# pennucci/PulsePortraiture

Measured on AMD Instinct MI355X. Metric: subint_fits_per_sec, higher is better.
Workload: dtype f64

## Files before the change

### pulseportraiture_amd/csrc/pp_fftq.h

```cpp
#pragma once
#include "pp_fft.h"

namespace pp {

__device__ __forceinline__ void lane_swap32(double& a, double& b) {
    unsigned alo = (unsigned)__double2loint(a), ahi = (unsigned)__double2hiint(a);
    unsigned blo = (unsigned)__double2loint(b), bhi = (unsigned)__double2hiint(b);
    auto r0 = __builtin_amdgcn_permlane32_swap(alo, blo, false, false);
    auto r1 = __builtin_amdgcn_permlane32_swap(ahi, bhi, false, false);
    a = __hiloint2double((int)r1[0], (int)r0[0]);
    b = __hiloint2double((int)r1[1], (int)r0[1]);
}
__device__ __forceinline__ void lane_swap16(double& a, double& b) {
    unsigned alo = (unsigned)__double2loint(a), ahi = (unsigned)__double2hiint(a);
    unsigned blo = (unsigned)__double2loint(b), bhi = (unsigned)__double2hiint(b);
    auto r0 = __builtin_amdgcn_permlane16_swap(alo, blo, false, false);
    auto r1 = __builtin_amdgcn_permlane16_swap(ahi, bhi, false, false);
    a = __hiloint2double((int)r1[0], (int)r0[0]);
    b = __hiloint2double((int)r1[1], (int)r0[1]);
}

__device__ __forceinline__ int fftq_lambda(int t) { return 4 * (t >> 4) + (t & 3) + 16 * ((t >> 2) & 3); }
__device__ __forceinline__ int fftq_lane_of(int lam) { return 16 * ((lam >> 2) & 3) + (lam & 3) + 4 * ((lam >> 4) & 3); }

constexpr int FFTQ_LDS_ELEMS = 4 * 272;

template <int WHEN = 0, typename Mid>
__device__ __forceinline__ void fftq1024(cplx (&v)[16], cplx* lds, const cplx t1, const cplx t2, int tid,
                                         double* power, Mid mid) {
    dft16_first(v);
    if (WHEN == 0) mid();
    dft16_second(v);
    {
        cplx wq[16];
        wq[1] = t1;
#pragma unroll
        for (int j = 2; j < 16; ++j) {
            if (j % 2 == 0) {
                const cplx h = wq[j / 2];
                wq[j] = make_double2(fma(h.x, h.x, -h.y * h.y), 2.0 * h.x * h.y);
            } else wq[j] = cmul(wq[j - 1], wq[1]);
        }
#pragma unroll
        for (int j = 1; j < 16; ++j) v[j] = cmul(v[j], wq[j]);
    }
    if (WHEN == 1) mid();
#pragma unroll
    for (int j = 0; j < 8; ++j) {
        lane_swap32(v[j].x, v[j + 8].x);
        lane_swap32(v[j].y, v[j + 8].y);
    }
#pragma unroll
    for (int j = 0; j < 16; ++j) {
        if (j & 4) continue;
        lane_swap16(v[j].x, v[j + 4].x);
        lane_swap16(v[j].y, v[j + 4].y);
    }
    if (WHEN == 2) mid();
    dft16_first(v);
    {
        const cplx w2 = make_double2(fma(t2.x, t2.x, -t2.y * t2.y), 2.0 * t2.x * t2.y);
        const cplx w3 = cmul(w2, t2);
#pragma unroll
        for (int c = 0; c < 4; ++c) {
            v[4 + c] = cmul(v[4 + c], t2);
            v[8 + c] = cmul(v[8 + c], w2);
            v[12 + c] = cmul(v[12 + c], w3);
        }
    }
    {
        cplx* wbase = lds + (tid >> 4) * 272 + 17 * (tid & 15);
#pragma unroll
        for (int j = 0; j < 16; ++j) wbase[j] = v[j];
        lds_sync<64>();
        const cplx* rbase = lds + (tid >> 4) * 272 + (tid & 15);
#pragma unroll
        for (int j = 0; j < 16; ++j) v[j] = rbase[17 * j];
        lds_sync<64>();
    }
    if (WHEN == 3) mid();
    dft_reg<16>(v);
    if (power) {
        double acc = 0.0;
#pragma unroll
        for (int j = 0; j < 16; ++j) {
            if (j == 0 && tid == 0) { const double dM = v[0].x - v[0].y; acc += dM * dM; }
            else acc += cnorm(v[j]);
        }
        *power += acc;
    }
}

__device__ __forceinline__ int fftq512_lambda(int t) {
    return 4 * ((t >> 5) & 1) + 2 * ((t >> 4) & 1) + 32 * ((t >> 3) & 1) + 16 * ((t >> 2) & 1) + 8 * ((t >> 1) & 1) + (t & 1);
}
__device__ __forceinline__ int fftq512_lane_of(int lam) {
    return 32 * ((lam >> 2) & 1) + 16 * ((lam >> 1) & 1) + 8 * ((lam >> 5) & 1) + 4 * ((lam >> 4) & 1) + 2 * ((lam >> 3) & 1) + (lam & 1);
}
constexpr int FFTQ512_LDS_ELEMS = 8 * 72;

__device__ __forceinline__ double lane_xor8(double v) {
    int lo = __double2loint(v), hi = __double2hiint(v);
    lo = __builtin_amdgcn_update_dpp(lo, lo, 0x128, 0xF, 0xF, false);
    hi = __builtin_amdgcn_update_dpp(hi, hi, 0x128, 0xF, 0xF, false);
    return __hiloint2double(hi, lo);
}

template <int WHEN = 0, typename Mid>
__device__ __forceinline__ void fftq512(cplx (&v)[8], cplx* lds, const cplx t1, const cplx t2, const cplx t3, int tid,
                                        double* power, Mid mid) {
    dft_reg<8>(v);
    if (WHEN == 0) mid();
    {
        cplx wq[8];
        wq[1] = t1;
#pragma unroll
        for (int j = 2; j < 8; ++j) {
            if (j % 2 == 0) {
                const cplx h = wq[j / 2];
                wq[j] = make_double2(fma(h.x, h.x, -h.y * h.y), 2.0 * h.x * h.y);
            } else wq[j] = cmul(wq[j - 1], wq[1]);
        }
#pragma unroll
        for (int j = 1; j < 8; ++j) v[j] = cmul(v[j], wq[j]);
    }
#pragma unroll
    for (int j = 0; j < 4; ++j) {
        lane_swap32(v[j].x, v[j + 4].x);
        lane_swap32(v[j].y, v[j + 4].y);
    }
#pragma unroll
    for (int j = 0; j < 8; ++j) {
        if (j & 2) continue;
        lane_swap16(v[j].x, v[j + 2].x);
        lane_swap16(v[j].y, v[j + 2].y);
    }
    dft4(v[0], v[2], v[4], v[6]);
    dft4(v[1], v[3], v[5], v[7]);
    {
        const cplx w2 = make_double2(fma(t2.x, t2.x, -t2.y * t2.y), 2.0 * t2.x * t2.y);
        const cplx w3 = cmul(w2, t2);
#pragma unroll
        for (int c = 0; c < 2; ++c) {
            v[2 + c] = cmul(v[2 + c], t2);
            v[4 + c] = cmul(v[4 + c], w2);
            v[6 + c] = cmul(v[6 + c], w3);
        }
    }
    {
        const bool up = (tid & 8) != 0;
        const double sg = up ? -1.0 : 1.0;
        const cplx w = up ? t3 : make_double2(1.0, 0.0);
#pragma unroll
        for (int j = 0; j < 8; ++j) {
            const cplx p = make_double2(lane_xor8(v[j].x), lane_xor8(v[j].y));
            const cplx d = make_double2(fma(sg, v[j].x, p.x), fma(sg, v[j].y, p.y));
            v[j] = cmul(d, w);
        }
    }
    {
        cplx* wbase = lds + (tid >> 3) * 72 + 9 * (tid & 7);
#pragma unroll
        for (int j = 0; j < 8; ++j) wbase[j] = v[j];
        lds_sync<64>();
        const cplx* rbase = lds + (tid >> 3) * 72 + (tid & 7);
#pragma unroll
        for (int j = 0; j < 8; ++j) v[j] = rbase[9 * j];
        lds_sync<64>();
    }
    if (WHEN == 3) mid();
    dft_reg<8>(v);
    if (power) {
        double acc = 0.0;
#pragma unroll
        for (int j = 0; j < 8; ++j) {
            if (j == 0 && tid == 0) { const double dM = v[0].x - v[0].y; acc += dM * dM; }
            else acc += cnorm(v[j]);
        }
        *power += acc;
    }
}

template <int M> struct FftQ;
template <> struct FftQ<1024> {
    static constexpr int R = 16, LDS_ELEMS = FFTQ_LDS_ELEMS;
    static __device__ __forceinline__ int lambda(int t) { return fftq_lambda(t); }
    static __device__ __forceinline__ int lane_of(int lam) { return fftq_lane_of(lam); }
    template <int WHEN, typename Mid>
    static __device__ __forceinline__ void run(cplx (&v)[16], cplx* lds, const cplx* twB, int tid, double* power, Mid mid) {
        const cplx t1 = twB[2 * tid], t2 = twB[32 * (tid & 15)];
        fftq1024<WHEN>(v, lds, t1, t2, tid, power, mid);
    }
};
template <> struct FftQ<512> {
    static constexpr int R = 8, LDS_ELEMS = FFTQ512_LDS_ELEMS;
    static __device__ __forceinline__ int lambda(int t) { return fftq512_lambda(t); }
    static __device__ __forceinline__ int lane_of(int lam) { return fftq512_lane_of(lam); }
    template <int WHEN, typename Mid>
    static __device__ __forceinline__ void run(cplx (&v)[8], cplx* lds, const cplx* twB, int tid, double* power, Mid mid) {
        const cplx t1 = twB[2 * tid], t2 = twB[16 * (tid & 15)], t3 = twB[64 * (tid & 7)];
        fftq512<WHEN>(v, lds, t1, t2, t3, tid, power, mid);
    }
};

}
```

### pulseportraiture_amd/csrc/pp_xspec1024q.h

```cpp
#pragma once
#ifndef PP_TAIL_M_LDS
#define PP_TAIL_M_LDS 1
#endif
#ifndef PP_MAIN_M_LDS
#define PP_MAIN_M_LDS 0
#endif
#include "pp_fftq.h"

#ifndef PP_SLOT_EARLY_EXIT
#define PP_SLOT_EARLY_EXIT 1
#endif
#ifndef PP_TICKET_SPREAD
#define PP_TICKET_SPREAD 0
#endif
#ifndef PP_TICKET_WINDOW_NUM
#define PP_TICKET_WINDOW_NUM 3u
#define PP_TICKET_WINDOW_DEN 4u
#endif
#ifndef PP_TAIL_HOOKS
#define PP_TAIL_HOOKS 1
#endif
#ifndef PP_SLOT_PUBLISH_KEPT
#define PP_SLOT_PUBLISH_KEPT 0
#endif

namespace pp {

constexpr bool Q_SPLIT_PREFETCH = true, Q_TW_RELOAD = true;
constexpr int Q_PREFETCH_F64 = 1, Q_PREFETCH_F32 = 0;
template <typename Tin, bool TAIL>
__global__ __launch_bounds__(64, 2) void k_xspec_q1024(XspecArgs a) {
    constexpr int M = 1024, T = 64, R1 = 16, PER1 = 1;
    constexpr int NSL = 7;
    typedef typename RawOf<Tin>::type Raw;
    constexpr int NRED = PP_TSTRIDE + (TAIL ? 2 : 1);
    static_assert(NRED <= 16, "wave_reduce_lds takes 16 values");
    static_assert(PP_TJ == 10, "power ladder written for order 10");
    constexpr int WRED = PP_WRED_DOUBLES(NRED) / 2;
    constexpr int LDSN = WRED > FFTQ_LDS_ELEMS ? WRED : FFTQ_LDS_ELEMS;
    static_assert(2 * LDSN >= PP_TAIL_LDS_DOUBLES, "tail_work's layout of this kernel's LDS");
    constexpr int NML = ((PP_TAIL_M_LDS && TAIL) || (PP_MAIN_M_LDS && !TAIL)) && sizeof(Tin) == 8 ? 2 : 0;
    __shared__ cplx lds[LDSN + 64 * NML];
    cplx* const ldsm = lds + LDSN + threadIdx.x;
    int tid = threadIdx.x;
    const long long nrows = (long long)a.nsub * a.nchan;
    Raw cur[PER1][R1];
    constexpr bool TWR = Q_TW_RELOAD && sizeof(Tin) == 8;
    cplx t1 = a.twB[2 * tid], t2 = a.twB[32 * (tid & 15)];
    const int lam0 = fftq_lambda(tid);
    cplx wb0 = a.twB[lam0 ? lam0 : 64];
    const cplx wbT = a.twB[64];
    int tail_after = 0x7fffffff;
    if (PP_TAIL_HOOKS && a.tail) {
        const unsigned share = (unsigned)(nrows / (long long)gridDim.x) + 1u;
        tail_after = 1 + (int)(((blockIdx.x * 2654435761u) >> 8) % (share * PP_TICKET_WINDOW_NUM / PP_TICKET_WINDOW_DEN + 1u));
#if PP_TICKET_SPREAD
        {
            const unsigned nt = (unsigned)a.tail_nsub;
            const unsigned div = nt ? gridDim.x / nt : 1u;
            if (div > 1u && (((blockIdx.x * 2246822519u) >> 11) % div) != 0u) tail_after = 0x7fffffff;
        }
#endif
    }
    RowWalk<true> rw;
    rw.start(nrows, a.mwords, a.ticket, a.ticket_base);
    long long row = rw.row;
    int n = 0, i = 0;
    if (rw.more) {
        n = __builtin_amdgcn_readfirstlane((int)(row / a.nsub));
        i = __builtin_amdgcn_readfirstlane((int)(row % a.nsub));
        const size_t rc = (size_t)sub_of(a.act, i) * a.nchan_full + (a.coff + n * a.cstep);
        stage_load_global<M, T, R1>(cur, reinterpret_cast<const Tin*>(a.data) + rc * (2 * M), tid);
    }
    cplx mv2[NSL];
    const cplx* mheld = nullptr;
    const cplx* mrow = nullptr;
    int n_held = -1, ktn = 0;
    int i_nx = i, n_nx = n;
#pragma unroll 1
    for (int phase = 0; phase < 2; ++phase) {
    if (phase == 1) {
        if (!(PP_TAIL_HOOKS && a.tail)) break;
        tail_work(a.tail, reinterpret_cast<double*>(lds), 2 * (LDSN + 64 * NML), tid, 1);
        tail_after = 0x7fffffff;
    }
    for (; rw.more && tail_after != 0; rw.advance(), row = rw.row, i = i_nx, n = n_nx, --tail_after) {
        rw.draw(a.ticket);
        rw.peek(nrows, a.ticket_base, a.mwords);
        asm volatile("" : "+v"(tid));
        const int lam = fftq_lambda(tid);
        const bool l0 = (lam == 0);
        const int kb = l0 ? 64 : lam;
        if (TWR) {
            t1 = as_global(a.twB)[2 * tid];
            t2 = as_global(a.twB)[32 * (tid & 15)];
            wb0 = as_global(a.twB)[kb];
        } else {
            asm volatile("" : "+v"(t1.x), "+v"(t1.y), "+v"(t2.x), "+v"(t2.y), "+v"(wb0.x), "+v"(wb0.y));
        }
        const int ia = sub_of(a.act, i), ne = a.coff + n * a.cstep;
        const size_t rc = (size_t)ia * a.nchan_full + ne;
        if (channel_lookup(a, ia, n, ne, M, n_held, mrow, ktn) && mrow != mheld) {
#pragma unroll
            for (int j = 0; j < NSL; ++j) {
                const cplx mval = mrow[kb + 64 * j - 1];
                if (j < NSL - NML) mv2[j] = mval; else ldsm[64 * (j - (NSL - NML))] = mval;
            }
            mheld = mrow;
        }
        const double phin = a.ph0[rc];
        double sd = 0.0;
        cplx v[R1];
#pragma unroll
        for (int k = 0; k < R1; ++k) v[k] = to_cplx(cur[0][k]);
        constexpr bool HALVES = Q_SPLIT_PREFETCH && sizeof(Tin) == 8;
        const Tin* nxrow = nullptr;
        auto load_some = [&](int k0, int k1) {
            const char* gb = reinterpret_cast<const char*>(nxrow);
            const unsigned boff = (unsigned)tid * (unsigned)sizeof(Raw);
#pragma unroll
            for (int k = 0; k < R1; ++k)
                if (k >= k0 && k < k1)
                    cur[0][k] = load_row_once<Raw>(gb + (size_t)(k * 64) * sizeof(Raw) + boff);
        };
#ifndef PP_NEXT_IN_LAMBDA
        rw.next(i, n, i_nx, n_nx, nrows, a.nsub, a.ticket_base, a.ticket, a.mwords);
        {
            const size_t rn = rw.more_nx
                ? (size_t)sub_of(a.act, i_nx) * a.nchan_full + (a.coff + n_nx * a.cstep) : rc;
            nxrow = reinterpret_cast<const Tin*>(a.data) + rn * (2 * M);
        }
#endif
        auto prefetch = [&]() {
            __builtin_amdgcn_sched_barrier(0);
#ifdef PP_NEXT_IN_LAMBDA
            rw.next(i, n, i_nx, n_nx, nrows, a.nsub, a.ticket_base, a.ticket, a.mwords);
            const size_t rn = rw.more_nx
                ? (size_t)sub_of(a.act, i_nx) * a.nchan_full + (a.coff + n_nx * a.cstep) : rc;
            nxrow = reinterpret_cast<const Tin*>(a.data) + rn * (2 * M);
#endif
            load_some(0, HALVES ? R1 / 2 : R1);
            __builtin_amdgcn_sched_barrier(0);
        };
        fftq1024<(sizeof(Tin) == 8 ? Q_PREFETCH_F64 : Q_PREFETCH_F32)>(v, lds, t1, t2, tid, &sd, prefetch);
        __builtin_amdgcn_sched_barrier(0);
        {
            cplx* pub = lds + tid;
            const int nk = PP_SLOT_PUBLISH_KEPT ? max(1, min(NSL, __builtin_amdgcn_readfirstlane(ktn) >> 6)) : NSL;
            switch (NSL - nk) {
                case 0: pub[64 * 0] = v[9];  [[fallthrough]];
                case 1: pub[64 * 1] = v[10]; [[fallthrough]];
                case 2: pub[64 * 2] = v[11]; [[fallthrough]];
                case 3: pub[64 * 3] = v[12]; [[fallthrough]];
                case 4: pub[64 * 4] = v[13]; [[fallthrough]];
                case 5: pub[64 * 5] = v[14]; [[fallthrough]];
                default: pub[64 * 6] = v[15];
            }
            static_assert(NSL == 7, "the run of stores above is written for seven slots");
            if (TAIL) {
#pragma unroll
                for (int r = 0; r < 5; ++r) pub[64 * (NSL + r)] = v[r];
            }
            lds_sync<T>();
        }
        double tail = 0.0;
        if (TAIL) {
            const double h = 0.70710678118654752440;
            const cplx* pt = lds + fftq_lane_of((64 - lam) & 63) + (l0 ? 64 : 0);
            cplx wt = l0 ? make_double2(-h, -h) : cmul(wb0, make_double2(-h, -h));
#pragma unroll
            for (int kd = 12; kd < 16; ++kd) {
                const cplx zk = v[kd];
                cplx zc = pt[64 * (NSL + 15 - kd)];
                zc.y = -zc.y;
                const cplx E = make_double2(zk.x + zc.x, zk.y + zc.y);
                const cplx O = make_double2(zk.x - zc.x, zk.y - zc.y);
                const cplx wo = cmul(wt, O);
                tail += cnorm(make_double2(E.x + wo.y, E.y - wo.x));
                wt = cmul(wt, wbT);
            }
            tail *= 0.25;
            if (tid == 0) { const double dM = v[0].x - v[0].y; tail += dM * dM; }
        }
        if (HALVES) {
            __builtin_amdgcn_sched_barrier(0);
            load_some(R1 / 2, R1);
            __builtin_amdgcn_sched_barrier(0);
        }
        const cplx* pc = lds + fftq_lane_of((64 - lam) & 63);
        const cplx el = unit_phasor<true>((double)kb, phin);
        const cplx wst = make_double2(bcast_lane0(el.x), bcast_lane0(el.y));
        cplx e = el, wb = wb0;
        const int ktu = __builtin_amdgcn_readfirstlane(ktn);
        const double kap0 = PP_TWO_PI * (double)kb;
        double tm[PP_TSTRIDE];
        cplx zc_nx = pc[64 * 6];
#pragma unroll
        for (int j = 0; j < NSL; ++j) {
            if (PP_SLOT_EARLY_EXIT && j > 0 && !(64 * j < ktu)) break;
            cplx zc = zc_nx;
            if (j + 1 < NSL && (!PP_SLOT_EARLY_EXIT || 64 * (j + 1) < ktu)) zc_nx = pc[64 * (5 - j)];
            if (j == 0 || 64 * j < ktu) {
                const cplx zk = csel(l0, v[j + 1], v[j]);
                zc.y = -zc.y;
                const cplx E = make_double2(zk.x + zc.x, zk.y + zc.y);
                const cplx O = make_double2(zk.x - zc.x, zk.y - zc.y);
                const cplx wo = cmul(wb, O);
                const cplx mj = (j < NSL - NML) ? mv2[j < NSL - NML ? j : 0] : ldsm[64 * (j - (NSL - NML))];
                const cplx x = cmulc(make_double2(E.x + wo.y, E.y - wo.x), mj);
                const cplx z = cmul(x, e);
                const double kap = j == 0 ? kap0 : kap0 + kconst<true>(PP_TWO_PI * (double)(64 * j));
                const double p2 = kap * kap, p4 = p2 * p2, p6 = p4 * p2, p8 = p4 * p4, p10 = p8 * p2;
                const double ui = z.y * kap;
                const double ax = fabs(x.x) + fabs(x.y);
                if (j == 0) {
                    tm[0] = z.x;
                    tm[1] = ui;
                    tm[2] = p2 * z.x;
                    tm[3] = p2 * ui;
                    tm[4] = p4 * z.x;
                    tm[5] = p4 * ui;
                    tm[6] = p6 * z.x;
                    tm[7] = p6 * ui;
                    tm[8] = p8 * z.x;
                    tm[9] = p8 * ui;
                    tm[10] = p10 * z.x;
                    tm[11] = (p10 * kap) * ax;
                } else {
                    tm[0] += z.x;
                    tm[1] += ui;
                    tm[2] = fma(p2, z.x, tm[2]);
                    tm[3] = fma(p2, ui, tm[3]);
                    tm[4] = fma(p4, z.x, tm[4]);
                    tm[5] = fma(p4, ui, tm[5]);
                    tm[6] = fma(p6, z.x, tm[6]);
                    tm[7] = fma(p6, ui, tm[7]);
                    tm[8] = fma(p8, z.x, tm[8]);
                    tm[9] = fma(p8, ui, tm[9]);
                    tm[10] = fma(p10, z.x, tm[10]);
                    tm[11] = fma(p10 * kap, ax, tm[11]);
                }
            }
            if (!PP_SLOT_EARLY_EXIT || (j + 1 < NSL && 64 * (j + 1) < ktu)) {
                wb = cmul(wb, wbT);
                e = cmul(e, wst);
            }
        }
        double tr[NRED];
#pragma unroll
        for (int j = 0; j < PP_TSTRIDE; ++j) tr[j] = tm[j];
        tr[PP_TSTRIDE] = sd;
        if (TAIL) tr[NRED - 1] = tail;
        lds_sync<T>();
        double tv = wave_reduce_lds(tr, tid, reinterpret_cast<double*>(lds));
        if ((tid & 3) == 0) {
            const int q = wave_reduce16_index(tid);
            if (q < PP_TSTRIDE) {
                tv *= 0.5;
                a.tay[tay_idx(rc, q)] = (q <= PP_TJ && ((q & 3) == 1 || (q & 3) == 2)) ? -tv : tv;
            }
        }
        if (tid == 4 * PP_TSTRIDE) a.sdraw[rc] = tv;
        if (TAIL && tid == 4 * (PP_TSTRIDE + 1)) {
            constexpr int H = M + 1, kc = (int)(0.75 * H);
            a.noise[rc] = sqrt(tv / (2.0 * M) / (double)(H - kc));
        }
        lds_sync<T>();
    }
    }
    if (PP_TAIL_HOOKS && a.tail) tail_work(a.tail, reinterpret_cast<double*>(lds), 2 * (LDSN + 64 * NML), tid, 1 << 30);
}


#ifndef PP_QF512_HOLD_TEMPLATE
#define PP_QF512_HOLD_TEMPLATE 1
#endif
#ifndef PP_QF512_WPS
#define PP_QF512_WPS 3
#endif
template <int M, typename Tin, bool TAIL>
__global__ __launch_bounds__(64, (M == 1024 ? 2 : PP_QF512_WPS)) void k_xspec_qf(XspecArgs a) {
    typedef FftQ<M> Q;
    constexpr int T = 64, R1 = Q::R, PER1 = 1;
    constexpr int NSL = R1;
    constexpr int JT = (3 * NSL) / 4;
    static_assert((int)(0.75 * (M + 1)) == 64 * JT, "the noise tail starts on a slot boundary");
    typedef typename RawOf<Tin>::type Raw;
    constexpr int NRED = PP_TSTRIDE + (TAIL ? 2 : 1);
    constexpr int WRED = PP_WRED_DOUBLES(NRED) / 2;
    constexpr int LDSN0 = Q::LDS_ELEMS > 64 * NSL ? Q::LDS_ELEMS : 64 * NSL;
    constexpr int LDSN = WRED > LDSN0 ? WRED : LDSN0;
    static_assert(M != 1024 || 2 * LDSN >= PP_TAIL_LDS_DOUBLES, "tail_work's layout of this kernel's LDS");
    __shared__ cplx lds[LDSN];
    int tid = threadIdx.x;
    const long long nrows = (long long)a.nsub * a.nchan;
    Raw cur[PER1][R1];
    const cplx wbT = a.twB[64];
    int tail_after = 0x7fffffff;
    if (PP_TAIL_HOOKS && M == 1024 && a.tail) {
        const unsigned share = (unsigned)(nrows / (long long)gridDim.x) + 1u;
        tail_after = 1 + (int)(((blockIdx.x * 2654435761u) >> 8) % (share * PP_TICKET_WINDOW_NUM / PP_TICKET_WINDOW_DEN + 1u));
    }
    RowWalk<true> rw;
    rw.start(nrows, a.mwords, a.ticket, a.ticket_base);
    long long row = rw.row;
    int n = 0, i = 0;
    if (rw.more) {
        n = __builtin_amdgcn_readfirstlane((int)(row / a.nsub));
        i = __builtin_amdgcn_readfirstlane((int)(row % a.nsub));
        const size_t rc = (size_t)sub_of(a.act, i) * a.nchan_full + (a.coff + n * a.cstep);
        stage_load_global<M, T, R1>(cur, reinterpret_cast<const Tin*>(a.data) + rc * (2 * M), tid);
    }
    int i_nx = i, n_nx = n;
    const cplx* mrow = nullptr;
    int n_held = -1, ktn = 0;
    constexpr bool MHOLD = PP_QF512_HOLD_TEMPLATE && M == 512;
    cplx mv[NSL];
    const cplx* mheld = nullptr;
#pragma unroll 1
    for (int phase = 0; phase < 2; ++phase) {
    if (phase == 1) {
        if (!(PP_TAIL_HOOKS && M == 1024 && a.tail)) break;
        tail_work(a.tail, reinterpret_cast<double*>(lds), 2 * LDSN, tid, 1);
        tail_after = 0x7fffffff;
    }
    for (; rw.more && tail_after != 0; rw.advance(), row = rw.row, i = i_nx, n = n_nx, --tail_after) {
        rw.draw(a.ticket);
        rw.peek(nrows, a.ticket_base, a.mwords);
        asm volatile("" : "+v"(tid));
        const int lam = Q::lambda(tid);
        const bool l0 = (lam == 0);
        const int kb = l0 ? 64 : lam;
        const cplx wb0 = as_global(a.twB)[kb];
        const int ia = sub_of(a.act, i), ne = a.coff + n * a.cstep;
        const size_t rc = (size_t)ia * a.nchan_full + ne;
        const bool looked = channel_lookup(a, ia, n, ne, M, n_held, mrow, ktn);
        if (MHOLD && looked && mrow != mheld) {
#pragma unroll
            for (int j = 0; j < NSL; ++j) mv[j] = mrow[kb + 64 * j - 1];
            mheld = mrow;
        }
        const double phin = a.ph0[rc];
        double sd = 0.0;
        cplx v[R1];
#pragma unroll
        for (int k = 0; k < R1; ++k) v[k] = to_cplx(cur[0][k]);
        auto template_loads = [&]() {
            if (MHOLD) return;
            __builtin_amdgcn_sched_barrier(0);
#pragma unroll
            for (int j = 0; j < NSL; ++j) mv[j] = mrow[kb + 64 * j - 1];
            __builtin_amdgcn_sched_barrier(0);
        };
        Q::template run<3>(v, lds, as_global(a.twB), tid, &sd, template_loads);
        __builtin_amdgcn_sched_barrier(0);
        {
            cplx* pub = lds + tid;
#pragma unroll
            for (int s = 0; s < NSL; ++s) pub[64 * s] = v[s];
            lds_sync<T>();
        }
        const Tin* nxrow;
        auto load_some = [&](int k0, int k1) {
            const char* gb = reinterpret_cast<const char*>(nxrow);
            const unsigned boff = (unsigned)tid * (unsigned)sizeof(Raw);
#pragma unroll
            for (int k = 0; k < R1; ++k)
                if (k >= k0 && k < k1) cur[0][k] = load_row_once<Raw>(gb + (size_t)(k * 64) * sizeof(Raw) + boff);
        };
        {
            __builtin_amdgcn_sched_barrier(0);
            rw.next(i, n, i_nx, n_nx, nrows, a.nsub, a.ticket_base, a.ticket, a.mwords);
            const size_t rn = rw.more_nx
                ? (size_t)sub_of(a.act, i_nx) * a.nchan_full + (a.coff + n_nx * a.cstep) : rc;
            nxrow = reinterpret_cast<const Tin*>(a.data) + rn * (2 * M);
            load_some(0, R1 / 2);
            __builtin_amdgcn_sched_barrier(0);
        }
        const cplx* pc = lds + Q::lane_of((64 - lam) & 63);
        const cplx el = unit_phasor<true>((double)kb, phin);
        const cplx wst = make_double2(bcast_lane0(el.x), bcast_lane0(el.y));
        cplx e = el, wb = wb0;
        const int ktu = __builtin_amdgcn_readfirstlane(ktn);
        const double kap0 = PP_TWO_PI * (double)kb;
        double tm[PP_TSTRIDE];
        double tail = 0.0;
        cplx zc_nx = pc[64 * (NSL - 1)];
#pragma unroll
        for (int j = 0; j < NSL; ++j) {
            if (PP_SLOT_EARLY_EXIT && !TAIL && j > NSL / 2 && !(64 * j < ktu)) break;
            cplx zc = zc_nx;
            if (j + 1 < NSL && (!PP_SLOT_EARLY_EXIT || TAIL || 64 * (j + 1) < ktu)) zc_nx = pc[64 * (NSL - 2 - j)];
            if (j == NSL / 2) {
                __builtin_amdgcn_sched_barrier(0);
                load_some(R1 / 2, R1);
                __builtin_amdgcn_sched_barrier(0);
            }
            const bool keep = (j == 0 || 64 * j < ktu);
            if (keep || (TAIL && j >= JT - 1)) {
                const cplx zk = csel(l0, v[(j + 1) & (NSL - 1)], v[j]);
                zc.y = -zc.y;
                const cplx E = make_double2(zk.x + zc.x, zk.y + zc.y);
                const cplx O = make_double2(zk.x - zc.x, zk.y - zc.y);
                const cplx wo = cmul(wb, O);
                const cplx dd = make_double2(E.x + wo.y, E.y - wo.x);
                if (TAIL && j >= JT - 1) {
                    const double pw = cnorm(dd);
                    tail += (j >= JT || l0) ? pw : 0.0;
                }
              if (keep) {
                const cplx x = cmulc(dd, mv[j]);
                const cplx z = cmul(x, e);
                const double kap = j == 0 ? kap0 : kap0 + kconst<true>(PP_TWO_PI * (double)(64 * j));
                const double p2 = kap * kap, p4 = p2 * p2, p6 = p4 * p2, p8 = p4 * p4, p10 = p8 * p2;
                const double ui = z.y * kap;
                const double ax = fabs(x.x) + fabs(x.y);
                if (j == 0) {
                    tm[0] = z.x;
                    tm[1] = ui;
                    tm[2] = p2 * z.x;
                    tm[3] = p2 * ui;
                    tm[4] = p4 * z.x;
                    tm[5] = p4 * ui;
                    tm[6] = p6 * z.x;
                    tm[7] = p6 * ui;
                    tm[8] = p8 * z.x;
                    tm[9] = p8 * ui;
                    tm[10] = p10 * z.x;
                    tm[11] = (p10 * kap) * ax;
                } else {
                    tm[0] += z.x;
                    tm[1] += ui;
                    tm[2] = fma(p2, z.x, tm[2]);
                    tm[3] = fma(p2, ui, tm[3]);
                    tm[4] = fma(p4, z.x, tm[4]);
                    tm[5] = fma(p4, ui, tm[5]);
                    tm[6] = fma(p6, z.x, tm[6]);
                    tm[7] = fma(p6, ui, tm[7]);
                    tm[8] = fma(p8, z.x, tm[8]);
                    tm[9] = fma(p8, ui, tm[9]);
                    tm[10] = fma(p10, z.x, tm[10]);
                    tm[11] = fma(p10 * kap, ax, tm[11]);
                }
              }
            }
            if (!PP_SLOT_EARLY_EXIT || TAIL || (j + 1 < NSL && 64 * (j + 1) < ktu)) {
                wb = cmul(wb, wbT);
                e = cmul(e, wst);
            }
        }
        double tr[NRED];
#pragma unroll
        for (int j = 0; j < PP_TSTRIDE; ++j) tr[j] = tm[j];
        tr[PP_TSTRIDE] = sd;
        if (TAIL) tr[NRED - 1] = 0.25 * tail;
        lds_sync<T>();
        double tv = wave_reduce_lds(tr, tid, reinterpret_cast<double*>(lds));
        if ((tid & 3) == 0) {
            const int q = wave_reduce16_index(tid);
            if (q < PP_TSTRIDE) {
                tv *= 0.5;
                a.tay[tay_idx(rc, q)] = (q <= PP_TJ && ((q & 3) == 1 || (q & 3) == 2)) ? -tv : tv;
            }
        }
        if (tid == 4 * PP_TSTRIDE) a.sdraw[rc] = tv;
        if (TAIL && tid == 4 * (PP_TSTRIDE + 1)) {
            constexpr int H = M + 1, kc = (int)(0.75 * H);
            a.noise[rc] = sqrt(tv / (2.0 * M) / (double)(H - kc));
        }
        lds_sync<T>();
    }
    }
    if (PP_TAIL_HOOKS && M == 1024 && a.tail) tail_work(a.tail, reinterpret_cast<double*>(lds), 2 * LDSN, tid, 1 << 30);
}

}
```

Before: 73840.

## Keep per-lane twiddles in LDS, scalarize row loads, and unify result stores

Per-lane twiddle constants (t1, t2, wb0) move into otherwise-unused LDS slots and are reloaded lazily inside the FFT instead of living in VGPRs or being re-fetched from global memory each row. The aim is to lower register pressure and global load traffic. The per-row phase load becomes a uniform (scalar) load, and the first row is awaited once before the loop. The scattered conditional result writes are merged into a single predicated global store per lane. These changes add LDS reads and barriers and depend on the reused LDS region staying free of row data.

Result: faster. 75190, median of 6 (+1.8%).

```diff
diff --git a/pulseportraiture_amd/csrc/pp_fftq.h b/pulseportraiture_amd/csrc/pp_fftq.h
--- a/pulseportraiture_amd/csrc/pp_fftq.h
+++ b/pulseportraiture_amd/csrc/pp_fftq.h
@@ -25,11 +25,12 @@
 
 constexpr int FFTQ_LDS_ELEMS = 4 * 272;
 
-template <int WHEN = 0, typename Mid>
-__device__ __forceinline__ void fftq1024(cplx (&v)[16], cplx* lds, const cplx t1, const cplx t2, int tid,
-                                         double* power, Mid mid) {
+template <int WHEN = 0, typename T1, typename T2, typename Mid>
+__device__ __forceinline__ void fftq1024_from(cplx (&v)[16], cplx* lds, T1 get_t1, T2 get_t2, int tid,
+                                              double* power, Mid mid) {
     dft16_first(v);
     if (WHEN == 0) mid();
+    const cplx t1 = get_t1();
     dft16_second(v);
     {
         cplx wq[16];
@@ -45,6 +46,7 @@
         for (int j = 1; j < 16; ++j) v[j] = cmul(v[j], wq[j]);
     }
     if (WHEN == 1) mid();
+    const cplx t2 = get_t2();
 #pragma unroll
     for (int j = 0; j < 8; ++j) {
         lane_swap32(v[j].x, v[j + 8].x);
@@ -89,6 +91,12 @@
         }
         *power += acc;
     }
+}
+
+template <int WHEN = 0, typename Mid>
+__device__ __forceinline__ void fftq1024(cplx (&v)[16], cplx* lds, const cplx t1, const cplx t2, int tid,
+                                         double* power, Mid mid) {
+    fftq1024_from<WHEN>(v, lds, [&]() { return t1; }, [&]() { return t2; }, tid, power, mid);
 }
 
 __device__ __forceinline__ int fftq512_lambda(int t) {
diff --git a/pulseportraiture_amd/csrc/pp_xspec1024q.h b/pulseportraiture_amd/csrc/pp_xspec1024q.h
--- a/pulseportraiture_amd/csrc/pp_xspec1024q.h
+++ b/pulseportraiture_amd/csrc/pp_xspec1024q.h
@@ -24,7 +24,62 @@
 #define PP_SLOT_PUBLISH_KEPT 0
 #endif
 
+#ifndef PP_LANE_CONSTS_LDS
+#define PP_LANE_CONSTS_LDS 1
+#endif
+#ifndef PP_TAIL_T2_LDS
+#define PP_TAIL_T2_LDS 0
+#endif
+#ifndef PP_TAIL_ROW_TOP
+#define PP_TAIL_ROW_TOP 0
+#endif
+#ifndef PP_ROW_WAIT_CEILING
+#define PP_ROW_WAIT_CEILING 0
+#endif
+
 namespace pp {
+
+constexpr int FFTQ_FREE_ELEM0 = 3 * 272 + 16, FFTQ_FREE_PITCH = 17;
+
+#ifndef PP_ROW_RESULTS_ONE_STORE
+#define PP_ROW_RESULTS_ONE_STORE 1
+#endif
+template <int M, bool TAIL, bool ONE = true>
+__device__ __forceinline__ void store_row_results(const XspecArgs& a, const size_t rc, const int tid, double tv) {
+    constexpr int H = M + 1, kc = (int)(0.75 * H);
+  if constexpr (ONE && PP_ROW_RESULTS_ONE_STORE) {
+    const int q = wave_reduce16_index(tid);
+    const double th = 0.5 * tv;
+    double val = (q <= PP_TJ && ((q & 3) == 1 || (q & 3) == 2)) ? -th : th;
+    double* dst = a.tay + tay_idx(rc, q < PP_TSTRIDE ? q : 0);
+    if (q >= PP_TSTRIDE) { val = tv; dst = a.sdraw + rc; }
+    if (TAIL) {
+        const double nz = sqrt(tv / (2.0 * M) / (double)(H - kc));
+        if (q > PP_TSTRIDE) { val = nz; dst = a.noise + rc; }
+    }
+    typedef double __attribute__((address_space(1)))* gdp_t;
+    *(gdp_t)(uintptr_t)dst = val;
+  } else {
+    if ((tid & 3) == 0) {
+        const int q = wave_reduce16_index(tid);
+        if (q < PP_TSTRIDE) {
+            tv *= 0.5;
+            a.tay[tay_idx(rc, q)] = (q <= PP_TJ && ((q & 3) == 1 || (q & 3) == 2)) ? -tv : tv;
+        }
+    }
+    if (tid == 4 * PP_TSTRIDE) a.sdraw[rc] = tv;
+    if (TAIL && tid == 4 * (PP_TSTRIDE + 1)) a.noise[rc] = sqrt(tv / (2.0 * M) / (double)(H - kc));
+  }
+}
+
+#ifndef PP_FIRST_ROW_LANDED
+#define PP_FIRST_ROW_LANDED 1
+#endif
+__device__ __forceinline__ void first_row_landed() {
+#if PP_FIRST_ROW_LANDED
+    __builtin_amdgcn_s_waitcnt(0x0F70);
+#endif
+}
 
 constexpr bool Q_SPLIT_PREFETCH = true, Q_TW_RELOAD = true;
 constexpr int Q_PREFETCH_F64 = 1, Q_PREFETCH_F32 = 0;
@@ -40,7 +95,13 @@
     constexpr int LDSN = WRED > FFTQ_LDS_ELEMS ? WRED : FFTQ_LDS_ELEMS;
     static_assert(2 * LDSN >= PP_TAIL_LDS_DOUBLES, "tail_work's layout of this kernel's LDS");
     constexpr int NML = ((PP_TAIL_M_LDS && TAIL) || (PP_MAIN_M_LDS && !TAIL)) && sizeof(Tin) == 8 ? 2 : 0;
-    __shared__ cplx lds[LDSN + 64 * NML];
+    constexpr bool TWL = PP_LANE_CONSTS_LDS && !PP_ROW_WAIT_CEILING && Q_TW_RELOAD && sizeof(Tin) == 8 && (!TAIL || PP_TAIL_T2_LDS);
+    constexpr bool ROWTOP = !TAIL || PP_TAIL_ROW_TOP;
+    constexpr int NTW = (TWL && NML == 0) ? 2 : 0;
+    __shared__ cplx lds[LDSN + 64 * (NML + NTW)];
+    static_assert(sizeof(lds) <= 19456, "eight workgroups per CU");
+    static_assert(FFTQ_FREE_ELEM0 + 15 * FFTQ_FREE_PITCH < FFTQ_LDS_ELEMS && FFTQ_FREE_ELEM0 >= 64 * (TAIL ? 12 : 7) &&
+                  2 * FFTQ_FREE_ELEM0 >= PP_WRED_DOUBLES(NRED), "t2's elements are outside everything a row writes");
     cplx* const ldsm = lds + LDSN + threadIdx.x;
     int tid = threadIdx.x;
     const long long nrows = (long long)a.nsub * a.nchan;
@@ -50,6 +111,15 @@
     const int lam0 = fftq_lambda(tid);
     cplx wb0 = a.twB[lam0 ? lam0 : 64];
     const cplx wbT = a.twB[64];
+    cplx* const ldt2 = lds + FFTQ_FREE_ELEM0;
+    cplx* const ldtw = lds + LDSN + 64 * NML;
+    auto put_lane_consts = [&](const cplx p1, const cplx p2, const cplx pb) {
+        if (!TWL) return;
+        ldt2[FFTQ_FREE_PITCH * (tid & 15)] = p2;
+        if (NTW) { ldtw[tid] = p1; ldtw[64 + tid] = pb; }
+        lds_sync<T>();
+    };
+    put_lane_consts(t1, t2, wb0);
     int tail_after = 0x7fffffff;
     if (PP_TAIL_HOOKS && a.tail) {
         const unsigned share = (unsigned)(nrows / (long long)gridDim.x) + 1u;
@@ -77,12 +147,17 @@
     const cplx* mrow = nullptr;
     int n_held = -1, ktn = 0;
     int i_nx = i, n_nx = n;
+    if (ROWTOP) first_row_landed();
 #pragma unroll 1
     for (int phase = 0; phase < 2; ++phase) {
     if (phase == 1) {
         if (!(PP_TAIL_HOOKS && a.tail)) break;
         tail_work(a.tail, reinterpret_cast<double*>(lds), 2 * (LDSN + 64 * NML), tid, 1);
         tail_after = 0x7fffffff;
+        if (TWL) {
+            const int lamr = fftq_lambda(tid);
+            put_lane_consts(as_global(a.twB)[2 * tid], as_global(a.twB)[32 * (tid & 15)], as_global(a.twB)[lamr ? lamr : 64]);
+        }
     }
     for (; rw.more && tail_after != 0; rw.advance(), row = rw.row, i = i_nx, n = n_nx, --tail_after) {
         rw.draw(a.ticket);
@@ -91,7 +166,12 @@
         const int lam = fftq_lambda(tid);
         const bool l0 = (lam == 0);
         const int kb = l0 ? 64 : lam;
-        if (TWR) {
+        if (PP_ROW_WAIT_CEILING && TWR) {
+            t1 = t2 = wb0 = wbT;
+            asm volatile("" : "+v"(t1.x), "+v"(t1.y), "+v"(t2.x), "+v"(t2.y), "+v"(wb0.x), "+v"(wb0.y));
+        } else if (TWL) {
+            if (!NTW) { t1 = as_global(a.twB)[2 * tid]; wb0 = as_global(a.twB)[kb]; }
+        } else if (TWR) {
             t1 = as_global(a.twB)[2 * tid];
             t2 = as_global(a.twB)[32 * (tid & 15)];
             wb0 = as_global(a.twB)[kb];
@@ -108,7 +188,7 @@
             }
             mheld = mrow;
         }
-        const double phin = a.ph0[rc];
+        const double phin = ROWTOP ? load_uniform(a.ph0 + rc) : a.ph0[rc];
         double sd = 0.0;
         cplx v[R1];
 #pragma unroll
@@ -142,7 +222,9 @@
             load_some(0, HALVES ? R1 / 2 : R1);
             __builtin_amdgcn_sched_barrier(0);
         };
-        fftq1024<(sizeof(Tin) == 8 ? Q_PREFETCH_F64 : Q_PREFETCH_F32)>(v, lds, t1, t2, tid, &sd, prefetch);
+        fftq1024_from<(sizeof(Tin) == 8 ? Q_PREFETCH_F64 : Q_PREFETCH_F32)>(
+            v, lds, [&]() { return NTW ? ldtw[tid] : t1; }, [&]() { return TWL ? ldt2[FFTQ_FREE_PITCH * (tid & 15)] : t2; },
+            tid, &sd, prefetch);
         __builtin_amdgcn_sched_barrier(0);
         {
             cplx* pub = lds + tid;
@@ -163,6 +245,7 @@
             }
             lds_sync<T>();
         }
+        if (NTW) wb0 = ldtw[64 + tid];
         double tail = 0.0;
         if (TAIL) {
             const double h = 0.70710678118654752440;
@@ -253,18 +336,7 @@
         if (TAIL) tr[NRED - 1] = tail;
         lds_sync<T>();
         double tv = wave_reduce_lds(tr, tid, reinterpret_cast<double*>(lds));
-        if ((tid & 3) == 0) {
-            const int q = wave_reduce16_index(tid);
-            if (q < PP_TSTRIDE) {
-                tv *= 0.5;
-                a.tay[tay_idx(rc, q)] = (q <= PP_TJ && ((q & 3) == 1 || (q & 3) == 2)) ? -tv : tv;
-            }
-        }
-        if (tid == 4 * PP_TSTRIDE) a.sdraw[rc] = tv;
-        if (TAIL && tid == 4 * (PP_TSTRIDE + 1)) {
-            constexpr int H = M + 1, kc = (int)(0.75 * H);
-            a.noise[rc] = sqrt(tv / (2.0 * M) / (double)(H - kc));
-        }
+        store_row_results<M, TAIL, ROWTOP>(a, rc, tid, tv);
         lds_sync<T>();
     }
     }
@@ -274,6 +346,12 @@
 
 #ifndef PP_QF512_HOLD_TEMPLATE
 #define PP_QF512_HOLD_TEMPLATE 1
+#endif
+#ifndef PP_QF_ROW_TOP
+#define PP_QF_ROW_TOP 1
+#endif
+#ifndef PP_QF_ROW_TOP_ALL
+#define PP_QF_ROW_TOP_ALL 0
 #endif
 #ifndef PP_QF512_WPS
 #define PP_QF512_WPS 3
@@ -293,6 +371,7 @@
     static_assert(M != 1024 || 2 * LDSN >= PP_TAIL_LDS_DOUBLES, "tail_work's layout of this kernel's LDS");
     __shared__ cplx lds[LDSN];
     int tid = threadIdx.x;
+    constexpr bool QTOP = PP_QF_ROW_TOP && ((M == 1024 && !TAIL) || PP_QF_ROW_TOP_ALL);
     const long long nrows = (long long)a.nsub * a.nchan;
     Raw cur[PER1][R1];
     const cplx wbT = a.twB[64];
@@ -317,6 +396,7 @@
     constexpr bool MHOLD = PP_QF512_HOLD_TEMPLATE && M == 512;
     cplx mv[NSL];
     const cplx* mheld = nullptr;
+    if (QTOP) first_row_landed();
 #pragma unroll 1
     for (int phase = 0; phase < 2; ++phase) {
     if (phase == 1) {
@@ -340,7 +420,7 @@
             for (int j = 0; j < NSL; ++j) mv[j] = mrow[kb + 64 * j - 1];
             mheld = mrow;
         }
-        const double phin = a.ph0[rc];
+        const double phin = QTOP ? load_uniform(a.ph0 + rc) : a.ph0[rc];
         double sd = 0.0;
         cplx v[R1];
 #pragma unroll
@@ -456,18 +536,7 @@
         if (TAIL) tr[NRED - 1] = 0.25 * tail;
         lds_sync<T>();
         double tv = wave_reduce_lds(tr, tid, reinterpret_cast<double*>(lds));
-        if ((tid & 3) == 0) {
-            const int q = wave_reduce16_index(tid);
-            if (q < PP_TSTRIDE) {
-                tv *= 0.5;
-                a.tay[tay_idx(rc, q)] = (q <= PP_TJ && ((q & 3) == 1 || (q & 3) == 2)) ? -tv : tv;
-            }
-        }
-        if (tid == 4 * PP_TSTRIDE) a.sdraw[rc] = tv;
-        if (TAIL && tid == 4 * (PP_TSTRIDE + 1)) {
-            constexpr int H = M + 1, kc = (int)(0.75 * H);
-            a.noise[rc] = sqrt(tv / (2.0 * M) / (double)(H - kc));
-        }
+        store_row_results<M, TAIL, QTOP>(a, rc, tid, tv);
         lds_sync<T>();
     }
     }
```
